# UltronAI/Depth-VO-Feat

Hardware: AMD Instinct MI355X
Metric: KITTI 256x832 stereo-seq samples/sec fwd+bwd (higher is better)
Workload: dtype f32

## Files before the change

### depth-vo-feat_amd/PoseExpNet.py

```python
from PoseExpNet_sfm import _PoseExpBase


class PoseExpNet(_PoseExpBase):

    def __init__(self, output_exp=True):
        super(PoseExpNet, self).__init__()
        self.nb_ref_imgs = 2
        self.output_exp = output_exp
        self._build(6, 6, self.nb_ref_imgs, output_exp)

    def forward(self, imgs):
        masks, pose = self._run(imgs)
        pose = pose.view(pose.size(0), 6)
        if self.training:
            return masks, pose
        return masks[0], pose
```

### depth-vo-feat_amd/PoseExpNet_sfm.py

```python
import torch
import torch.nn as nn

from dvf import lib as _L
from dvf.conv import FusedAct, FusedConv2d, FusedConvTranspose2d, SpatialMeanFn, xavier_init_

_ENC_PLANES = (16, 32, 64, 128, 256, 256, 256)
_ENC_KERNEL = (7, 5, 3, 3, 3, 3, 3)
_DEC_PLANES = (256, 128, 64, 32, 16)


class _PoseExpBase(nn.Module):

    def _build(self, in_planes, n_pose_out, nb_masks, output_exp):
        cin = in_planes
        for i, (co, k) in enumerate(zip(_ENC_PLANES, _ENC_KERNEL), start=1):
            setattr(self, f"conv{i}", nn.Sequential(FusedConv2d(cin, co, k, 2, (k - 1) // 2, _L.ACT_RELU, fuse_bwd=True), FusedAct()))
            cin = co
        self.pose_pred = FusedConv2d(_ENC_PLANES[6], n_pose_out, 1, 1, 0)
        if output_exp:
            up_in = (_ENC_PLANES[4],) + _DEC_PLANES[:-1]
            for j, lvl in enumerate(range(5, 0, -1)):
                setattr(self, f"upconv{lvl}", nn.Sequential(
                    FusedConvTranspose2d(up_in[j], _DEC_PLANES[j], 4, 2, 1, _L.ACT_RELU, fuse_bwd=True), FusedAct()))
            for lvl, ci in zip((4, 3, 2, 1), _DEC_PLANES[1:]):
                setattr(self, f"predict_mask{lvl}", FusedConv2d(ci, nb_masks, 3, 1, 1, _L.ACT_SIGMOID_AFFINE))

    def init_weights(self):
        xavier_init_(self)

    def _run(self, frames):
        outs = []
        h = frames
        for i in range(1, 8):
            h = getattr(self, f"conv{i}")[0](*h) if isinstance(h, (list, tuple)) else getattr(self, f"conv{i}")[0](h)
            outs.append(h)
        pose = SpatialMeanFn.apply(self.pose_pred(h), 0.01)
        masks = [None, None, None, None]
        if self.output_exp:
            first = frames[0] if isinstance(frames, (list, tuple)) else frames
            refs = [outs[3], outs[2], outs[1], outs[0], first]
            h = outs[4]
            ups = []
            for j, lvl in enumerate(range(5, 0, -1)):
                h = getattr(self, f"upconv{lvl}")[0](h, out_hw=(refs[j].size(2), refs[j].size(3)))
                ups.append(h)
            for lvl in (4, 3, 2, 1):
                masks[lvl - 1] = getattr(self, f"predict_mask{lvl}")(ups[5 - lvl])
        return masks, pose


class PoseExpNet(_PoseExpBase):

    def __init__(self, nb_ref_imgs=2, output_exp=True):
        super(PoseExpNet, self).__init__()
        self.nb_ref_imgs = nb_ref_imgs
        self.output_exp = output_exp
        self._build(3 * (1 + nb_ref_imgs), 6 * nb_ref_imgs, nb_ref_imgs, output_exp)

    def forward(self, target_image, ref_imgs):
        assert(len(ref_imgs) == self.nb_ref_imgs)
        frames = [target_image] + list(ref_imgs)
        if len(frames) > _L.MAX_SEGS:
            raise ValueError(f"nb_ref_imgs = {self.nb_ref_imgs}: at most {_L.MAX_SEGS - 1} reference images are supported")
        masks, pose = self._run(frames)
        pose = pose.view(pose.size(0), self.nb_ref_imgs, 6)
        if self.training:
            return masks, pose
        return masks[0], pose
```

### depth-vo-feat_amd/csrc/conv.hip

```cpp
#include "dvf_common.h"
#include "conv_op.h"
#include "conv_pipe_host.h"
#include "conv_gather.h"
#include "conv_wgrad.h"
#include "wgrad_pipe.h"

namespace {

__device__ __forceinline__ float act_grad(float g, float yv, int act, float alpha, float beta) {
    if (act == DVF_ACT_RELU) return (yv > 0.f) ? g : 0.f;
    if (act == DVF_ACT_SIGMOID_AFFINE) {
        const float sg = (yv - beta) / alpha;
        return g * alpha * sg * (1.f - sg);
    }
    return g;
}

template <bool VEC>
__global__ __launch_bounds__(256) void act_bwd_kernel(const float *__restrict__ dy, const float *__restrict__ y,
                                                      float *__restrict__ dpre, float *dbias, int C, int HW, int act,
                                                      float alpha, float beta, int chunks, float *part = nullptr, int nper = 0) {
    __shared__ float red[4];
    const int plane = blockIdx.x / chunks, chunk = blockIdx.x - plane * chunks;
    const int c = plane % C;
    const int64_t base = (int64_t)plane * HW;
    float s = 0.f;
    if (VEC) {
        typedef float f4 __attribute__((ext_vector_type(4)));
        const int HW4 = HW >> 2, per = (HW4 + chunks - 1) / chunks;
        const int beg = chunk * per, end = min(HW4, beg + per);
        const f4 *dy4 = reinterpret_cast<const f4 *>(dy + base), *y4 = reinterpret_cast<const f4 *>(y ? y + base : dy + base);
        f4 *o4 = reinterpret_cast<f4 *>(dpre ? dpre + base : nullptr);
        for (int i0 = beg + threadIdx.x; i0 < end; i0 += 1024) {
            f4 g[4], yv[4];
#pragma unroll
            for (int k = 0; k < 4; ++k) {
                const int i = i0 + 256 * k;
                if (i < end) { g[k] = dy4[i]; yv[k] = (act != DVF_ACT_NONE) ? y4[i] : g[k]; }
            }
#pragma unroll
            for (int k = 0; k < 4; ++k) {
                const int i = i0 + 256 * k;
                if (i < end) {
                    f4 r;
#pragma unroll
                    for (int e = 0; e < 4; ++e) { r[e] = act_grad(g[k][e], yv[k][e], act, alpha, beta); s += r[e]; }
                    if (dpre) o4[i] = r;
                }
            }
        }
    } else {
        const int per = (HW + chunks - 1) / chunks;
        const int beg = chunk * per, end = min(HW, beg + per);
        for (int i = beg + threadIdx.x; i < end; i += 256) {
            const float g = act_grad(dy[base + i], (act != DVF_ACT_NONE) ? y[base + i] : 0.f, act, alpha, beta);
            if (dpre) dpre[base + i] = g;
            s += g;
        }
    }
    if (dbias) {
        s = wave_sum(s);
        if ((threadIdx.x & 63) == 0) red[threadIdx.x >> 6] = s;
        __syncthreads();
        if (threadIdx.x == 0) {
            const float t = (red[0] + red[1]) + (red[2] + red[3]);
            if (part) part[(int64_t)c * nper + (plane / C) * chunks + chunk] = t;
            else atomicAdd(&dbias[c], t);
        }
    }
}

__global__ __launch_bounds__(64) void bias_finish_kernel(const float *__restrict__ part, float *dbias, int n) {
    const float *p = part + (int64_t)blockIdx.x * n;
    float s = 0.f;
    for (int i = threadIdx.x; i < n; i += 64) s += p[i];
    s = wave_sum(s);
    if (threadIdx.x == 0) dbias[blockIdx.x] += s;
}

struct TilePlan { int lsw, lsh, TGX, TGY, NT; };

TilePlan plan_tiles(int OHc, int OWc, int NT, int maxBW = 64) {
    TilePlan best{5, 0, 1, 4 * NT, NT};
    double best_cost = 1e30;
    for (int lsw = 5; lsw >= 0; --lsw) {
        const int lsh = 5 - lsw, SW = 1 << lsw, SH = 1 << lsh;
        for (int TGX = 1; TGX <= 4 * NT; TGX *= 2) {
            const int TGY = 4 * NT / TGX, BW = TGX * SW, BH = TGY * SH;
            if (BW > maxBW) continue;
            const double cov = (double)cdiv(OWc, BW) * BW * cdiv(OHc, BH) * BH;
            const double cost = cov * (1.0 + 0.02 * lsh) + 1e-3 * (BW + BH);
            if (cost < best_cost) { best_cost = cost; best = TilePlan{lsw, lsh, TGX, TGY, NT}; }
        }
    }
    return best;
}

struct GatherPlan {
    GatherArgs a;
    int MT, NT, CKH;
    size_t lds;
    dim3 grid;
    int64_t ws_floats;
    bool reduce_kpar;
};

int plan_gather(const ConvOp &op, GatherPlan &pl) {
    const ClassSpec *cls = op.cls;
    const int ncls = op.ncls, Tmax = op.Tmax, TAmax = op.TAmax, TBmax = op.TBmax, OHc = op.OHc, OWc = op.OWc;
    if (ncls < 1 || ncls > 4) return DVF_ERR_INVALID_ARG;
    GatherArgs &a = pl.a;
    a = GatherArgs{};
    for (int s = 0; s < op.nseg; ++s) a.segC[s] = op.segC[s];
    a.nseg = op.nseg; a.w_mode = op.w_mode;
    a.Mtot = op.Mtot; a.Rtot = op.Rtot; a.KK = op.KK; a.m_base = op.m_base; a.M = op.M;
    a.N = op.N; a.IH = op.IH; a.IW = op.IW; a.OH = op.OH; a.OW = op.OW;
    a.act = op.act; a.alpha = op.alpha; a.beta = op.beta;
    a.ncls = ncls; a.OS = cls[0].OS; a.IS = cls[0].IS;
    for (int i = 0, tap0 = 0; i < ncls; ++i) {
        const ClassSpec &c = cls[i];
        const int T = c.TA * c.TB;
// ... 355 lines not shown

extern "C" {

int64_t dvf_conv2d_wgrad_ws_floats(const dvf_conv_desc *d, const int *seg_channels, int nseg) {
    int rc = check_desc(d);
    if (rc) return rc;
    rc = check_segs(d, seg_channels, nseg);
    if (rc) return rc;
    int64_t need = 0;
    if (dvf_head_applicable(d, nseg)) {
        need = dvf_head_wgrad_ws_floats(d);
    } else {
        const float *const none[DVF_MAX_SEGS] = {};
        WgradPipePlan pp;
        auto plan = [&](int s, const int *qsegc, int qnseg) {
            const WgradArgs a = wgrad_args(d, none, seg_channels, s, nullptr, nullptr);
            if (plan_wgrad_pipe(a, qsegc, qnseg, true, false, pp) == DVF_OK && pp.ws_floats > need) need = pp.ws_floats;
        };
        if (!d->transposed) plan(-1, seg_channels, nseg);
        else for (int s = 0; s < nseg; ++s) plan(s, &d->C_out, 1);
    }
    const int64_t nb = dvf_act_bwd_ws_floats(d->N, d->C_out, d->H_out * d->W_out);
    return need > nb ? need : nb;
}

int dvf_conv2d_wgrad(const dvf_conv_desc *d, const float *const *in_segs, const int *seg_channels, int nseg,
                     const float *dpre, float *dw, int accumulate, float *dbias, int accumulate_dbias, float *ws,
                     int64_t ws_floats, void *stream) {
    if (!d) return DVF_ERR_INVALID_ARG;
    hipStream_t st = dvf_stream(stream);
    if (dbias && !accumulate_dbias &&
        hipMemsetAsync(dbias, 0, sizeof(float) * (size_t)(d->C_out > 0 ? d->C_out : 0), st) != hipSuccess)
        return DVF_ERR_LAUNCH;
    dvf_plan_reset();
    int rc = check_desc(d);
    if (rc) return rc;
    rc = check_segs(d, seg_channels, nseg);
    if (rc) return rc;
    if (!in_segs || !dpre || !dw) return DVF_ERR_INVALID_ARG;
    bool done = false;
    rc = wgrad_route(d, in_segs, seg_channels, nseg, dpre, dw, accumulate, dbias, &done, ws, ws_floats, st);
    if (rc || done || !dbias) return rc;
    return dvf_act_bwd(dpre, nullptr, nullptr, dbias, d->N, d->C_out, d->H_out * d->W_out, DVF_ACT_NONE, 1.f, 0.f, 1, ws, ws_floats, stream);
}

static int act_bwd_chunks(int N, int C, int HW, bool has_bias) {
    int chunks = (HW + 8191) / 8192;
    const int64_t planes = (int64_t)N * C;
    while (chunks > 1 && planes * chunks > 16384) chunks >>= 1;
    while (planes * chunks < 1024 && HW / (chunks * 2) >= 1024 && (!has_bias || (int64_t)N * chunks * 2 <= 128)) chunks *= 2;
    return chunks;
}

int64_t dvf_act_bwd_ws_floats(int N, int C, int HW) {
    if (N <= 0 || C <= 0 || HW <= 0) return DVF_ERR_INVALID_ARG;
    return (int64_t)C * N * act_bwd_chunks(N, C, HW, true);
}

int dvf_act_bwd(const float *dy, const float *y, float *dpre, float *dbias, int N, int C, int HW, int act, float alpha,
                float beta, int accumulate_dbias, float *ws, int64_t ws_floats, void *stream) {
    if (!dy || (act != DVF_ACT_NONE && !y) || N <= 0 || C <= 0 || HW <= 0) return DVF_ERR_INVALID_ARG;
    if (!dpre && !dbias) return DVF_OK;
    hipStream_t st = dvf_stream(stream);
    if (dbias && !accumulate_dbias && hipMemsetAsync(dbias, 0, sizeof(float) * C, st) != hipSuccess) return DVF_ERR_LAUNCH;
    const bool vec = (HW % 4 == 0) && ((reinterpret_cast<uintptr_t>(dy) | reinterpret_cast<uintptr_t>(y) |
                                        reinterpret_cast<uintptr_t>(dpre)) % 16 == 0);
    const int chunks = act_bwd_chunks(N, C, HW, dbias != nullptr);
    const int64_t planes = (int64_t)N * C;
    float *part = (dbias && ws && ws_floats >= dvf_act_bwd_ws_floats(N, C, HW)) ? ws : nullptr;
    if (vec) act_bwd_kernel<true><<<(unsigned)(planes * chunks), 256, 0, st>>>(dy, y, dpre, dbias, C, HW, act, alpha, beta, chunks, part, N * chunks);
    else act_bwd_kernel<false><<<(unsigned)(planes * chunks), 256, 0, st>>>(dy, y, dpre, dbias, C, HW, act, alpha, beta, chunks, part, N * chunks);
    DVF_LAUNCH_CHECK();
    if (part) {
        bias_finish_kernel<<<C, 64, 0, st>>>(part, dbias, N * chunks);
        DVF_LAUNCH_CHECK();
    }
    return DVF_OK;
}


int64_t dvf_conv2d_packed_floats(const dvf_conv_desc *d, const int *seg_channels, int nseg, int op_kind) {
    return conv_sizes(d, seg_channels, nseg, op_kind, false);
}

int64_t dvf_conv2d_ws_floats(const dvf_conv_desc *d, const int *seg_channels, int nseg, int op_kind) {
    return conv_sizes(d, seg_channels, nseg, op_kind, true);
}

int dvf_conv2d_pack(const dvf_conv_desc *d, const int *seg_channels, int nseg, int op_kind, const float *w, float *packed,
                    void *stream) {
    int rc = check_desc(d);
    if (rc) return rc;
    rc = check_segs(d, seg_channels, nseg);
    if (rc) return rc;
    if (!w || !packed) return DVF_ERR_INVALID_ARG;
    hipStream_t st = dvf_stream(stream);
    if (op_kind == 0) {
        ConvOp op;
        PipePlan pl;
        rc = make_fwd_op(d, seg_channels, nseg, op);
        if (!rc) rc = plan_pipe(op, pl);
        return rc ? rc : launch_pack(op, pl, w, packed, st);
    }
    if (op_kind != 1) return DVF_ERR_INVALID_ARG;
    return for_each_dgrad_seg(d, seg_channels, nseg, true, [&](const DgradSeg &v) -> int {
        return v.packed ? launch_pack(v.op, v.plan, w, packed + v.packed_off, st) : DVF_OK;
    });
}

int dvf_conv2d_fwd(const dvf_conv_desc *d, const float *const *in_segs, const int *seg_channels, int nseg,
                   const float *packed, const float *w, const float *bias, float *out, float *ws, int64_t ws_floats,
                   void *stream) {
    dvf_plan_reset();
    int rc = check_desc(d);
    if (rc) return rc;
    rc = check_segs(d, seg_channels, nseg);
    if (rc) return rc;
    if (!in_segs || !w || !out) return DVF_ERR_INVALID_ARG;
    for (int s = 0; s < nseg; ++s)
        if (!in_segs[s]) return DVF_ERR_INVALID_ARG;
    hipStream_t st = dvf_stream(stream);
    const ConvIO io{in_segs, bias, out, nullptr};
    ConvOp op;
// ... 91 lines not shown
```

### depth-vo-feat_amd/csrc/conv_head.hip

```cpp
#include "conv_head.h"
#include "conv_epilogue.h"

namespace {

using dvfp::apply_act;

constexpr int HT_W = 64, HT_H = 4;
constexpr int HP_W = HT_W + 2, HP_H = HT_H + 2;
constexpr int HCK = 8;
constexpr int HWK = 7;

__device__ __forceinline__ void stage_tile(float *lds, const float *__restrict__ src, int64_t plane, int nch, int H, int W,
                                           int y0, int x0) {
    for (int e = threadIdx.x; e < nch * HP_H * HP_W; e += 256) {
        const int ch = e / (HP_H * HP_W), r = e - ch * (HP_H * HP_W), py = r / HP_W, px = r - py * HP_W;
        const int y = y0 + py - 1, x = x0 + px - 1;
        lds[e] = (y >= 0 && y < H && x >= 0 && x < W) ? src[ch * plane + (int64_t)y * W + x] : 0.f;
    }
}

template <int ROWS, int MO, class WK>
__device__ __forceinline__ void taps9(const float (&v)[ROWS + 2][3], WK wk, float (&acc)[ROWS][MO]) {
#pragma unroll
    for (int m = 0; m < MO; ++m)
#pragma unroll
        for (int k = 0; k < 9; ++k) {
            const float w = wk(m, k);
#pragma unroll
            for (int r = 0; r < ROWS; ++r) acc[r][m] = fmaf(w, v[k / 3 + r][k % 3], acc[r][m]);
        }
}

constexpr int FT_H = 8;
constexpr int HEAD_MAX_SEGS = 3;
struct HeadSegs {
    const float *p[HEAD_MAX_SEGS];
    int c[HEAD_MAX_SEGS];
    int n;
};
template <int MO, int HCKT, int FTH>
__global__ __launch_bounds__(256) void head_fwd_kernel(const HeadSegs in, const float *__restrict__ w,
                                                       const float *__restrict__ bias, float *__restrict__ out, int C, int H,
                                                       int W, int tilesX, int act, float alpha, float beta, int ws_m, int ws_c,
                                                       int flip, const float *__restrict__ mask) {
    constexpr int ROWS = FTH / 4, FPH = FTH + 2, FPN = FPH * HP_W, FLD = (FPN + 255) / 256;
    extern __shared__ __attribute__((aligned(16))) float wsh[];
    float *tile = wsh + ((MO * C * 9 + 3) & ~3);
    for (int e = threadIdx.x; e < MO * C * 9; e += 256) {
        const int m = e / (C * 9), r = e - m * (C * 9), c = r / 9, k = r - c * 9;
        const float wv = w[(int64_t)m * ws_m + (int64_t)c * ws_c + (flip ? 8 - k : k)];
        if (MO == 16) wsh[(c * MO + m) * 9 + k] = wv;
        else wsh[e] = wv;
    }
    const int n = blockIdx.y, tY = blockIdx.x / tilesX, tX = blockIdx.x - tY * tilesX;
    const int y0 = tY * FTH, x0 = tX * HT_W;
    const int lx = threadIdx.x & (HT_W - 1), ly = (threadIdx.x >> 6) * ROWS;
    const int64_t plane = (int64_t)H * W;
    int soff[FLD];
#pragma unroll
    for (int i = 0; i < FLD; ++i) {
        const int e = threadIdx.x + 256 * i, py = e / HP_W, px = e - py * HP_W;
        const int y = y0 + py - 1, x = x0 + px - 1;
        soff[i] = (e < FPN && y >= 0 && y < H && x >= 0 && x < W) ? y * W + x : -1;
// ... 112 lines not shown
        }
    }
}

template <int MO>
__global__ __launch_bounds__(256) void head_dgrad_kernel(const float *__restrict__ dpre, const float *__restrict__ w,
                                                         float *__restrict__ din, int C, int H, int W, int tilesX,
                                                         const float *__restrict__ mask) {
    __shared__ float tile[MO * HP_H * HP_W];
    extern __shared__ __attribute__((aligned(16))) float wsh[];
    constexpr int WPC = (MO * 9 + 3) & ~3;
    for (int e = threadIdx.x; e < C * MO * 9; e += 256) {
        const int c = e / (MO * 9), r = e - c * (MO * 9), m = r / 9, k = r - m * 9;
        wsh[c * WPC + r] = w[((int64_t)m * C + c) * 9 + k];
    }
    const int n = blockIdx.y, tY = blockIdx.x / tilesX, tX = blockIdx.x - tY * tilesX;
    const int y0 = tY * HT_H, x0 = tX * HT_W;
    const int lx = threadIdx.x & (HT_W - 1), ly = threadIdx.x >> 6;
    const int64_t plane = (int64_t)H * W;
    stage_tile(tile, dpre + (int64_t)n * MO * plane, plane, MO, H, W, y0, x0);
    __syncthreads();
    float g[MO][9];
#pragma unroll
    for (int m = 0; m < MO; ++m)
#pragma unroll
        for (int a = 0; a < 3; ++a)
#pragma unroll
            for (int b = 0; b < 3; ++b) g[m][a * 3 + b] = tile[m * (HP_H * HP_W) + (ly + 2 - a) * HP_W + (lx + 2 - b)];
    const int y = y0 + ly, x = x0 + lx;
    if (y >= H || x >= W) return;
    const int64_t base = (int64_t)n * C * plane + (int64_t)y * W + x;
    float *dst = din + base;
    const float *mk = mask ? mask + base : nullptr;
    for (int c0 = 0; c0 < C; c0 += 4) {
        float sv[4], mv[4];
#pragma unroll
        for (int q = 0; q < 4; ++q) {
            const int c = min(c0 + q, C - 1);
            mv[q] = mk ? mk[c * plane] : 1.f;
            const float *wc = wsh + c * WPC;
            float s = 0.f;
#pragma unroll
            for (int m = 0; m < MO; ++m)
#pragma unroll
                for (int k = 0; k < 9; ++k) s = fmaf(wc[m * 9 + k], g[m][k], s);
            sv[q] = s;
        }
#pragma unroll
        for (int q = 0; q < 4; ++q)
            if (c0 + q < C) dst[(c0 + q) * plane] = (mv[q] > 0.f) ? sv[q] : 0.f;
    }
}

template <int MO>
__global__ __launch_bounds__(256) void head_wgrad_kernel(const float *__restrict__ in, const float *__restrict__ dpre,
                                                         float *dw, int N, int C, int H, int W, int tilesX, int tilesY,
                                                         float *part = nullptr) {
    __shared__ float tin[HWK * HP_H * HP_W];
    __shared__ float tdp[MO * HT_H * HT_W];
    __shared__ float red[4 * HWK * 9 * MO];
    const int c0 = blockIdx.x * HWK, nch = min(HWK, C - c0);
    const int64_t plane = (int64_t)H * W;
    const int wave = threadIdx.x >> 6, lane = threadIdx.x & 63;
    const int col_c = lane / 9, col_t = lane - col_c * 9, ta = col_t / 3, tb = col_t - ta * 3;
    const bool active = lane < nch * 9;
    float acc[MO];
#pragma unroll
    for (int m = 0; m < MO; ++m) acc[m] = 0.f;
    const int ntiles = N * tilesX * tilesY;
    for (int tile = blockIdx.y; tile < ntiles; tile += gridDim.y) {
        const int n = tile / (tilesX * tilesY), r = tile - n * (tilesX * tilesY), tY = r / tilesX, tX = r - tY * tilesX;
        const int y0 = tY * HT_H, x0 = tX * HT_W;
        __syncthreads();
        stage_tile(tin, in + ((int64_t)n * C + c0) * plane, plane, nch, H, W, y0, x0);
        for (int e = threadIdx.x; e < MO * HT_H * HT_W; e += 256) {
            const int m = e / (HT_H * HT_W), q = e - m * (HT_H * HT_W), py = q / HT_W, px = q - py * HT_W;
            const int y = y0 + py, x = x0 + px;
            tdp[e] = (y < H && x < W) ? dpre[((int64_t)n * MO + m) * plane + (int64_t)y * W + x] : 0.f;
        }
        __syncthreads();
        if (active) {
            const float *src = tin + col_c * (HP_H * HP_W) + (wave + ta) * HP_W + tb;
            const float *dp = tdp + wave * HT_W;
#pragma unroll 8
            for (int px = 0; px < HT_W; ++px) {
                const float v = src[px];
#pragma unroll
                for (int m = 0; m < MO; ++m) acc[m] = fmaf(dp[m * (HT_H * HT_W) + px], v, acc[m]);
            }
        }
    }
    if (active)
#pragma unroll
        for (int m = 0; m < MO; ++m) red[(wave * MO + m) * (HWK * 9) + lane] = acc[m];
    __syncthreads();
    if (wave == 0 && active) {
#pragma unroll
        for (int m = 0; m < MO; ++m) {
            const float s = (red[(0 * MO + m) * (HWK * 9) + lane] + red[(1 * MO + m) * (HWK * 9) + lane]) +
                            (red[(2 * MO + m) * (HWK * 9) + lane] + red[(3 * MO + m) * (HWK * 9) + lane]);
            const int64_t o = ((int64_t)m * C + c0 + col_c) * 9 + col_t;
            if (part) part[(int64_t)blockIdx.y * MO * C * 9 + o] = s;
            else atomicAdd(&dw[o], s);
        }
    }
}

__global__ __launch_bounds__(256) void head_wgrad_finish_kernel(const float *__restrict__ part, float *dw, int n, int groups) {
    const int e = blockIdx.x * 256 + threadIdx.x;
    if (e >= n) return;
    float s = 0.f;
    for (int g = 0; g < groups; ++g) s += part[(int64_t)g * n + e];
    dw[e] += s;
}


template <int CO, int K>
__global__ __launch_bounds__(256) void dconvt_s2_fwd_kernel(const float *__restrict__ in, const float *__restrict__ w,
                                                            const float *__restrict__ bias, float *__restrict__ out, int C, int H,
                                                            int W, int OH, int OW, int act, float alpha, float beta) {
    extern __shared__ __attribute__((aligned(16))) float wlds[];
    constexpr int WPC = CO * K * K;
    static_assert(WPC % 4 == 0, "weights of one input channel are read in 16-byte pieces");
    typedef float f4w __attribute__((ext_vector_type(4)));
    for (int e = threadIdx.x; e < C * WPC / 4; e += 256)
        reinterpret_cast<f4w *>(wlds)[e] = reinterpret_cast<const f4w *>(w)[e];
    __syncthreads();
    const int x = blockIdx.x * 64 + (threadIdx.x & 63), y = blockIdx.y * 4 + (threadIdx.x >> 6), n = blockIdx.z;
    const bool inside = x < W && y < H;
    const bool rok[3] = {y - 1 >= 0 && y - 1 < H, y < H, y + 1 < H}, cok[3] = {x - 1 >= 0 && x - 1 < W, x < W, x + 1 < W};
    float acc[2][2][CO];
#pragma unroll
    for (int co = 0; co < CO; ++co) {
        const float b = bias ? bias[co] : 0.f;
        acc[0][0][co] = acc[0][1][co] = acc[1][0][co] = acc[1][1][co] = b;
    }
    const int64_t plane = (int64_t)H * W;
    const float *ip = in + (int64_t)n * C * plane + (int64_t)y * W + x;
    for (int ci = 0; ci < C; ++ci) {
        float v[3][3];
#pragma unroll
        for (int r = (K == 3 ? 1 : 0); r < 3; ++r)
#pragma unroll
            for (int c = (K == 3 ? 1 : 0); c < 3; ++c) v[r][c] = (rok[r] && cok[c]) ? ip[(r - 1) * W + (c - 1)] : 0.f;
        const f4w *wc = reinterpret_cast<const f4w *>(wlds + ci * WPC);
        f4w wq[WPC / 4];
#pragma unroll
        for (int q = 0; q < WPC / 4; ++q) wq[q] = wc[q];
#pragma unroll
        for (int co = 0; co < CO; ++co) {
#pragma unroll
            for (int a = 0; a < K; ++a) {
                const int dy = (a + 1) & 1;
                const int ry = 1 + ((dy + 1 - a) >> 1);
// ... 104 lines not shown
    const int one = d->C_in;
    return dvf_head_fwd_segs(d, &in, &one, 1, w, bias, out, st);
}

bool dvf_head_wide_applicable(const dvf_conv_desc *d, int nseg) {
    return nseg >= 1 && nseg <= HEAD_MAX_SEGS && !d->transposed && d->KH == 3 && d->KW == 3 && d->stride == 1 && d->pad == 1 &&
           d->C_out == 16 && d->C_in <= 24 && d->H_out == d->H_in && d->W_out == d->W_in &&
           (int64_t)d->H_in * d->W_in >= 64 * 64 && dvf_tune("DVF_NO_HEAD") == nullptr && dvf_tune("DVF_NO_WIDE_HEAD") == nullptr;
}

int dvf_head_fwd_segs(const dvf_conv_desc *d, const float *const *in_segs, const int *seg_channels, int nseg, const float *w,
                      const float *bias, float *out, hipStream_t st) {
    HeadSegs in{};
    for (int s = 0; s < HEAD_MAX_SEGS; ++s) { in.p[s] = s < nseg ? in_segs[s] : in_segs[0]; in.c[s] = s < nseg ? seg_channels[s] : 0; }
    in.n = nseg;
    const int rc = head_fwd_launch(d->C_out, in, w, bias, out, d->C_in, d->N, d->H_in, d->W_in, d->act, d->alpha, d->beta,
                                   d->C_in * 9, 9, 0, nullptr, st);
    if (rc) return rc;
    dvf_plan_note(DVF_K_HEAD_FWD, d->C_out, nseg);
    return DVF_OK;
}

bool dvf_head_seg_dgrad_applicable(const dvf_conv_desc *d, int segc) {
    const bool narrow = segc >= 1 && segc <= 4 && d->C_out >= 4 && d->C_out * segc <= 1024;
    const bool wide = segc == 16 && d->C_out <= 24 && (int64_t)d->H_in * d->W_in >= 64 * 64 &&
                      dvf_tune("DVF_NO_WIDE_HEAD") == nullptr;
    return !d->transposed && d->KH == 3 && d->KW == 3 && d->stride == 1 && d->pad == 1 && (narrow || wide) &&
           d->H_out == d->H_in && d->W_out == d->W_in && dvf_tune("DVF_NO_HEAD") == nullptr;
}

int dvf_head_seg_dgrad(const dvf_conv_desc *d, const float *dpre, const float *w, float *din, int seg_off, int segc,
                       hipStream_t st, const float *mask) {
    const float *wseg = w + (int64_t)seg_off * 9;
    HeadSegs in{};
    for (int s = 0; s < HEAD_MAX_SEGS; ++s) { in.p[s] = dpre; in.c[s] = s == 0 ? d->C_out : 0; }
    in.n = 1;
    const int rc = head_fwd_launch(segc, in, wseg, nullptr, din, d->C_out, d->N, d->H_in, d->W_in, DVF_ACT_NONE, 1.f, 0.f, 9,
                                   d->C_in * 9, 1, mask, st);
    if (rc) return rc;
    dvf_plan_note(DVF_K_HEAD_SEG_DGRAD, segc);
    return DVF_OK;
}

int dvf_head_dgrad(const dvf_conv_desc *d, const float *dpre, const float *w, float *din, hipStream_t st, const float *mask) {
    const int tilesX = cdiv(d->W_in, HT_W), tilesY = cdiv(d->H_in, HT_H);
    const dim3 grid(tilesX * tilesY, d->N);
    HEAD_DISPATCH(d->C_out, (head_dgrad_kernel<MO><<<grid, 256, (size_t)d->C_in * ((MO * 9 + 3) & ~3) * 4, st>>>(
                                dpre, w, din, d->C_in, d->H_in, d->W_in, tilesX, mask)));
    DVF_LAUNCH_CHECK();
    dvf_plan_note(DVF_K_HEAD_DGRAD, d->C_out);
    return DVF_OK;
}

static void head_wgrad_grid(const dvf_conv_desc *d, int &tilesX, int &tilesY, int &chunks, int &groups) {
    tilesX = cdiv(d->W_in, HT_W); tilesY = cdiv(d->H_in, HT_H);
    chunks = cdiv(d->C_in, HWK);
    const int ntiles = d->N * tilesX * tilesY;
    groups = 2048 / chunks;
    if (groups < 1) groups = 1;
    if (groups > ntiles) groups = ntiles;
}

int64_t dvf_head_wgrad_ws_floats(const dvf_conv_desc *d) {
    int tilesX, tilesY, chunks, groups;
    head_wgrad_grid(d, tilesX, tilesY, chunks, groups);
    return (int64_t)groups * d->C_out * d->C_in * 9;
}

int dvf_head_wgrad(const dvf_conv_desc *d, const float *in, const float *dpre, float *dw, int accumulate, hipStream_t st,
                   float *ws, int64_t ws_floats) {
    if (!accumulate && hipMemsetAsync(dw, 0, sizeof(float) * (size_t)d->C_out * d->C_in * 9, st) != hipSuccess)
        return DVF_ERR_LAUNCH;
    int tilesX, tilesY, chunks, groups;
    head_wgrad_grid(d, tilesX, tilesY, chunks, groups);
    const dim3 grid(chunks, groups);
    float *part = (ws && ws_floats >= dvf_head_wgrad_ws_floats(d)) ? ws : nullptr;
    HEAD_DISPATCH(d->C_out, (head_wgrad_kernel<MO><<<grid, 256, 0, st>>>(in, dpre, dw, d->N, d->C_in, d->H_in, d->W_in, tilesX,
                                                                        tilesY, part)));
    DVF_LAUNCH_CHECK();
    if (part) {
        const int n = d->C_out * d->C_in * 9;
        head_wgrad_finish_kernel<<<(n + 255) / 256, 256, 0, st>>>(part, dw, n, groups);
        DVF_LAUNCH_CHECK();
    }
    dvf_plan_note(DVF_K_HEAD_WGRAD, d->C_out, part ? 1 : 0);
    return DVF_OK;
}
```

### depth-vo-feat_amd/dvf/steps.py

```python

import torch

import loss_functions as LF
import loss_functions_sfm as LS
from dvf import lib as L
from dvf.conv import reciprocal


POSE_STREAM = True


def _side_by_side(aux_fn, main_fn):
    if L.SERIALIZE or not POSE_STREAM:
        m_out = main_fn()
        return aux_fn(), m_out
    cur = torch.cuda.current_stream()
    aux = L.aux_stream(cur.device)
    aux.wait_stream(cur)
    m_out = main_fn()
    with torch.cuda.stream(aux):
        a_out = aux_fn()
    cur.wait_stream(aux)

    def _mark(t):
        if torch.is_tensor(t):
            t.record_stream(cur)
        elif isinstance(t, (list, tuple)):
            for x in t:
                _mark(x)
    _mark(a_out)
    return a_out, m_out


def _identity_share(counts, n_views):
    return counts[n_views:2 * n_views].sum() / counts.sum()


def unsupervise_losses(depth_net, pose_net, batch, feat_extractor=None, img_scale=0.004, smooth_weight=10.0,
                       feat_weight=0.1, depth_eps=1e-4, ssim_weight=0.0, ssim_c1=1e-4, ssim_c2=9e-4, min_reprojection=False,
                       auto_mask=False, normalized_smoothness=False):
    counts = []
    R2, R1, L2 = batch["img_R2"], batch["img_R1"], batch["img_L2"]
    (_, T_2to1), disps = _side_by_side(lambda: pose_net((R2, R1)), lambda: depth_net(R2))
    inv_depth = disps[0]
    depth = reciprocal(inv_depth, depth_eps).squeeze(1)
    img_loss = LF.photometric_reconstruction_loss(R2, R1, L2, depth, T_2to1, batch["T_R2L"], batch["K"], batch["Kinv"],
                                                  img_scale=img_scale,
                                                  ssim_weight=ssim_weight, ssim_c1=ssim_c1, ssim_c2=ssim_c2,
                                                  min_reprojection=min_reprojection, auto_mask=auto_mask,
                                                  selection_counts=counts)
    if normalized_smoothness:
        smooth = LF.normalized_smooth_loss(inv_depth, R2, img_scale=img_scale)
    else:
        smooth = LF.smooth_loss(depth.unsqueeze(1))
    terms = {"img": img_loss.detach(), "smooth": smooth.detach()}
    if auto_mask:
        terms["automask"] = _identity_share(counts[0], 2)
    loss = img_loss + smooth_weight * smooth
    if feat_extractor is not None:
        b = R2.size(0)
        feat = feat_extractor(torch.cat((L2, R2, R1), dim=0))
        f_L2, f_R2, f_R1 = feat[:b], feat[b:2 * b], feat[2 * b:]
        feat_loss = LF.photometric_reconstruction_loss(f_R2, f_R1, f_L2, depth, T_2to1, batch["T_R2L"], batch["K"],
                                                       batch["Kinv"])
        loss = img_loss + feat_weight * feat_loss + smooth_weight * smooth
        terms["feat"] = feat_loss.detach()
    terms["total"] = loss.detach()
    return loss, terms


def depth_only_losses(depth_net, batch, img_scale=0.004, smooth_weight=10.0, depth_eps=1e-4):
    R2, L2 = batch["img_R2"], batch["img_L2"]
    depth = reciprocal(depth_net(R2)[0], depth_eps)
    from dvf.ops import PhotoLossFn
    photo = PhotoLossFn.apply(R2, depth.squeeze(1), batch["T_R2L"].unsqueeze(0).contiguous(), batch["K"], batch["Kinv"], None,
                              (0, float(img_scale)), L2)
    smooth = LF.smooth_loss(depth)
    loss = photo + smooth_weight * smooth
    return loss, {"img": photo.detach(), "smooth": smooth.detach(), "total": loss.detach()}


def train_sfm_losses(disp_net, pose_exp_net, batch, w1=1.0, w2=0.0, w3=0.1, smooth_factor=2.0,
                     rotation_mode="euler", padding_mode="zeros", feat_extractor=None, feat_weight=0.1,
                     ssim_weight=0.0, ssim_c1=1e-4, ssim_c2=9e-4, min_reprojection=False, auto_mask=False,
                     full_res_multiscale=False, normalized_smoothness=False):
    if min_reprojection and w2 > 0:
        raise ValueError("min_reprojection leaves the explainability mask out of the photometric term: w2 must be 0")
    tgt = batch["img_R2"]
    refs = [batch["img_R1"], batch["img_L2"]] + list(batch.get("extra_refs", []))[: pose_exp_net.nb_ref_imgs - 2]
    (masks, pose), disparities = _side_by_side(lambda: pose_exp_net(tgt, refs), lambda: disp_net(tgt))
    depth = [reciprocal(d, 0.0) for d in disparities]
    counts = []
    photo_depth, photo_masks = depth, masks
    if full_res_multiscale:
        hw = tgt.shape[2:]
        photo_depth = LS.full_resolution(disparities, hw, recip_eps=0.0)
        if not min_reprojection:
            photo_masks = LS.full_resolution(masks, hw)
    l1 = LS.photometric_reconstruction_loss(tgt, refs, batch["K"], batch["Kinv"], photo_depth,
                                            [None] * len(depth) if min_reprojection else photo_masks, pose,
                                            rotation_mode, padding_mode, ssim_weight=ssim_weight, ssim_c1=ssim_c1,
                                            ssim_c2=ssim_c2, min_reprojection=min_reprojection, auto_mask=auto_mask,
                                            selection_counts=counts)
    if normalized_smoothness:
        l3 = LS.normalized_smooth_loss(disparities, tgt, smooth_factor)
    else:
        l3 = LS.smooth_loss(depth, smooth_factor)
    l4 = torch.nn.functional.mse_loss(pose[:, 1], batch["T_R2L"])
    loss = w1 * l1 + w3 * l3 + l4
    terms = {"photo": l1.detach(), "smooth": l3.detach(), "lr": l4.detach()}
    if auto_mask:
        terms["automask"] = _identity_share(counts[0], len(refs))
    if w2 > 0:
        l2 = LS.explainability_loss(masks)
        loss = loss + w2 * l2
        terms["exp"] = l2.detach()
    if feat_extractor is not None:
        b = tgt.size(0)
        feat = feat_extractor(torch.cat((refs[1], tgt, refs[0]), dim=0))
        f_L2, f_R2, f_R1 = feat[:b], feat[b:2 * b], feat[2 * b:]
        lf = LF.photometric_reconstruction_loss(f_R2, f_R1, f_L2, depth[0].squeeze(1), pose[:, 0], pose[:, 1], batch["K"],
                                                batch["Kinv"], rotation_mode, padding_mode)
        loss = loss + feat_weight * lf
        terms["feat"] = lf.detach()
    terms["total"] = loss.detach()
    return loss, terms


def unsupervise_dvo_losses(depth_net, pose_net, batch, img_scale=0.004, smooth_weight=10.0, depth_eps=1e-4,
                           normalized_smoothness=False):
    from dvf.ops import PhotoLossFn
    R2, R1, L2 = batch["img_R2"], batch["img_R1"], batch["img_L2"]
    (_, T_2to1), disps = _side_by_side(lambda: pose_net((R2, R1)), lambda: depth_net(R2))
    inv_depth = disps[0]
    depth = reciprocal(inv_depth, depth_eps)
    pose = torch.stack((batch["T_R2L"], T_2to1), dim=0)
    photo = PhotoLossFn.apply(R2, depth.squeeze(1), pose, batch["K"], batch["Kinv"], None,
                              (L.POSE_SE3 | L.PIXEL_COORDS, float(img_scale)), L2, R1)
    smooth = LF.normalized_smooth_loss(inv_depth, R2, img_scale=img_scale) if normalized_smoothness else LF.smooth_loss(depth)
    loss = photo + smooth_weight * smooth
    return loss, {"photo": photo.detach(), "smooth": smooth.detach(), "total": loss.detach()}


def paper_losses(depth_net, pose_net, batch, feat_extractor=None, img_scale=0.004, smooth_weight=10.0, feat_weight=0.1,
                 depth_eps=1e-4):
    import loss_functions_caffe as LC
    R2, R1, L2 = batch["img_R2"], batch["img_R1"], batch["img_L2"]
    (_, T_2to1), disps = _side_by_side(lambda: pose_net((R2, R1)), lambda: depth_net(R2))
    inv_depth = disps[0]
    depth = reciprocal(inv_depth, depth_eps)
    poses = (batch["T_R2L_se3"], T_2to1)
    photo = LC.abs_warp_loss(R2, (L2, R1), depth, poses, batch["K"], batch["Kinv"], img_scale=img_scale)
    smooth = LC.edge_aware_smooth_loss(inv_depth, R2, img_scale=img_scale)
    loss = photo + smooth_weight * smooth
    terms = {"photo": photo.detach(), "smooth": smooth.detach()}
    if feat_extractor is not None:
        b = R2.size(0)
        with torch.no_grad():
            feat = feat_extractor(torch.cat((L2, R2, R1), dim=0))
        f_L2, f_R2, f_R1 = feat[:b], feat[b:2 * b], feat[2 * b:]
        lf = LC.abs_warp_loss(f_R2, (f_L2, f_R1), depth, poses, batch["K"], batch["Kinv"])
        loss = loss + feat_weight * lf
        terms["feat"] = lf.detach()
    terms["total"] = loss.detach()
    return loss, terms
```

Before: 615.9.

## Skip unused mask decoder, add bias-sum kernel, rewrite head wgrad as register sliding window

The stereo-sequence loss paths now call the pose net with need_masks=False, so the upconv/mask decoder is not run when its masks are discarded. A dedicated wide bias-sum reduction kernel handles the bias-only backward case (no activation, no dpre) with its own chunking. The 3x3 head weight-gradient kernel is rewritten from LDS tiles into a per-thread register sliding window over row segments with vectorized loads and tunable channel and row grouping. Together these remove wasted forward/backward work and cut reduction overhead, at the cost of more registers and new tuning heuristics.

```diff
diff --git a/depth-vo-feat_amd/PoseExpNet.py b/depth-vo-feat_amd/PoseExpNet.py
--- a/depth-vo-feat_amd/PoseExpNet.py
+++ b/depth-vo-feat_amd/PoseExpNet.py
@@ -9,8 +9,8 @@
         self.output_exp = output_exp
         self._build(6, 6, self.nb_ref_imgs, output_exp)
 
-    def forward(self, imgs):
-        masks, pose = self._run(imgs)
+    def forward(self, imgs, need_masks=True):
+        masks, pose = self._run(imgs, need_masks)
         pose = pose.view(pose.size(0), 6)
         if self.training:
             return masks, pose
diff --git a/depth-vo-feat_amd/PoseExpNet_sfm.py b/depth-vo-feat_amd/PoseExpNet_sfm.py
--- a/depth-vo-feat_amd/PoseExpNet_sfm.py
+++ b/depth-vo-feat_amd/PoseExpNet_sfm.py
@@ -28,7 +28,7 @@
     def init_weights(self):
         xavier_init_(self)
 
-    def _run(self, frames):
+    def _run(self, frames, need_masks=True):
         outs = []
         h = frames
         for i in range(1, 8):
@@ -36,7 +36,7 @@
             outs.append(h)
         pose = SpatialMeanFn.apply(self.pose_pred(h), 0.01)
         masks = [None, None, None, None]
-        if self.output_exp:
+        if self.output_exp and need_masks:
             first = frames[0] if isinstance(frames, (list, tuple)) else frames
             refs = [outs[3], outs[2], outs[1], outs[0], first]
             h = outs[4]
@@ -57,12 +57,12 @@
         self.output_exp = output_exp
         self._build(3 * (1 + nb_ref_imgs), 6 * nb_ref_imgs, nb_ref_imgs, output_exp)
 
-    def forward(self, target_image, ref_imgs):
+    def forward(self, target_image, ref_imgs, need_masks=True):
         assert(len(ref_imgs) == self.nb_ref_imgs)
         frames = [target_image] + list(ref_imgs)
         if len(frames) > _L.MAX_SEGS:
             raise ValueError(f"nb_ref_imgs = {self.nb_ref_imgs}: at most {_L.MAX_SEGS - 1} reference images are supported")
-        masks, pose = self._run(frames)
+        masks, pose = self._run(frames, need_masks)
         pose = pose.view(pose.size(0), self.nb_ref_imgs, 6)
         if self.training:
             return masks, pose
diff --git a/depth-vo-feat_amd/csrc/conv.hip b/depth-vo-feat_amd/csrc/conv.hip
--- a/depth-vo-feat_amd/csrc/conv.hip
+++ b/depth-vo-feat_amd/csrc/conv.hip
@@ -67,6 +67,54 @@
             if (part) part[(int64_t)c * nper + (plane / C) * chunks + chunk] = t;
             else atomicAdd(&dbias[c], t);
         }
+    }
+}
+
+template <bool VEC>
+__global__ __launch_bounds__(1024) void bias_sum_kernel(const float *__restrict__ dy, float *dbias, int C, int HW, int chunks,
+                                                        float *part, int nper) {
+    __shared__ float red[16];
+    constexpr int U = 8, UT = 4;
+    typedef typename std::conditional<VEC, float __attribute__((ext_vector_type(4))), float>::type V;
+    const int T = blockDim.x;
+    const int plane = blockIdx.x / chunks, chunk = blockIdx.x - plane * chunks;
+    const int c = plane % C;
+    const int E = VEC ? HW >> 2 : HW, per = (E + chunks - 1) / chunks;
+    const int beg = chunk * per, n = min(E, beg + per) - beg;
+    const V *p = reinterpret_cast<const V *>(dy + (int64_t)plane * HW) + beg;
+    const V zero = {};
+    V a0 = zero, a1 = zero;
+    int i = threadIdx.x;
+    for (; i + T * (U - 1) < n; i += T * U) {
+        V g[U];
+#pragma unroll
+        for (int k = 0; k < U; ++k) g[k] = p[i + T * k];
+#pragma unroll
+        for (int k = 0; k < U; k += 2) { a0 += g[k]; a1 += g[k + 1]; }
+    }
+    for (; i < n; i += T * UT) {
+        V g[UT];
+#pragma unroll
+        for (int k = 0; k < UT; ++k) g[k] = p[min(i + T * k, n - 1)];
+#pragma unroll
+        for (int k = 0; k < UT; ++k) a0 += (i + T * k < n) ? g[k] : zero;
+    }
+    a0 += a1;
+    float s;
+    if constexpr (VEC) s = (a0[0] + a0[1]) + (a0[2] + a0[3]);
+    else s = a0;
+    s = wave_sum(s);
+    if (T > 64) {
+        if ((threadIdx.x & 63) == 0) red[threadIdx.x >> 6] = s;
+        __syncthreads();
+        if (threadIdx.x == 0) {
+            s = red[0];
+            for (int w = 1; w < (T >> 6); ++w) s += red[w];
+        }
+    }
+    if (threadIdx.x == 0) {
+        if (part) part[(int64_t)c * nper + (plane / C) * chunks + chunk] = s;
+        else atomicAdd(&dbias[c], s);
     }
 }
 
@@ -528,9 +576,18 @@
     return chunks;
 }
 
+static int bias_sum_chunks(int N, int C, int HW) {
+    int target = 256;
+    if (const char *t = dvf_tune("DVF_BIAS_BLOCKS")) target = atoi(t);
+    int chunks = 1;
+    while ((int64_t)N * C * chunks * 2 <= target && HW / (chunks * 2) >= 8192) chunks *= 2;
+    return chunks;
+}
+
 int64_t dvf_act_bwd_ws_floats(int N, int C, int HW) {
     if (N <= 0 || C <= 0 || HW <= 0) return DVF_ERR_INVALID_ARG;
-    return (int64_t)C * N * act_bwd_chunks(N, C, HW, true);
+    const int a = act_bwd_chunks(N, C, HW, true), b = bias_sum_chunks(N, C, HW);
+    return (int64_t)C * N * (a > b ? a : b);
 }
 
 int dvf_act_bwd(const float *dy, const float *y, float *dpre, float *dbias, int N, int C, int HW, int act, float alpha,
@@ -541,10 +598,16 @@
     if (dbias && !accumulate_dbias && hipMemsetAsync(dbias, 0, sizeof(float) * C, st) != hipSuccess) return DVF_ERR_LAUNCH;
     const bool vec = (HW % 4 == 0) && ((reinterpret_cast<uintptr_t>(dy) | reinterpret_cast<uintptr_t>(y) |
                                         reinterpret_cast<uintptr_t>(dpre)) % 16 == 0);
-    const int chunks = act_bwd_chunks(N, C, HW, dbias != nullptr);
+    const bool sums_only = !dpre && act == DVF_ACT_NONE;
+    const int chunks = sums_only ? bias_sum_chunks(N, C, HW) : act_bwd_chunks(N, C, HW, dbias != nullptr);
     const int64_t planes = (int64_t)N * C;
     float *part = (dbias && ws && ws_floats >= dvf_act_bwd_ws_floats(N, C, HW)) ? ws : nullptr;
-    if (vec) act_bwd_kernel<true><<<(unsigned)(planes * chunks), 256, 0, st>>>(dy, y, dpre, dbias, C, HW, act, alpha, beta, chunks, part, N * chunks);
+    if (sums_only) {
+        const int per = ((vec ? HW >> 2 : HW) + chunks - 1) / chunks;
+        const int threads = per <= 256 ? 64 : per <= 8192 ? 256 : 1024;
+        if (vec) bias_sum_kernel<true><<<(unsigned)(planes * chunks), threads, 0, st>>>(dy, dbias, C, HW, chunks, part, N * chunks);
+        else bias_sum_kernel<false><<<(unsigned)(planes * chunks), threads, 0, st>>>(dy, dbias, C, HW, chunks, part, N * chunks);
+    } else if (vec) act_bwd_kernel<true><<<(unsigned)(planes * chunks), 256, 0, st>>>(dy, y, dpre, dbias, C, HW, act, alpha, beta, chunks, part, N * chunks);
     else act_bwd_kernel<false><<<(unsigned)(planes * chunks), 256, 0, st>>>(dy, y, dpre, dbias, C, HW, act, alpha, beta, chunks, part, N * chunks);
     DVF_LAUNCH_CHECK();
     if (part) {
diff --git a/depth-vo-feat_amd/csrc/conv_head.hip b/depth-vo-feat_amd/csrc/conv_head.hip
--- a/depth-vo-feat_amd/csrc/conv_head.hip
+++ b/depth-vo-feat_amd/csrc/conv_head.hip
@@ -8,7 +8,6 @@
 constexpr int HT_W = 64, HT_H = 4;
 constexpr int HP_W = HT_W + 2, HP_H = HT_H + 2;
 constexpr int HCK = 8;
-constexpr int HWK = 7;
 
 __device__ __forceinline__ void stage_tile(float *lds, const float *__restrict__ src, int64_t plane, int nch, int H, int W,
                                            int y0, int x0) {
@@ -227,54 +226,114 @@
     }
 }
 
-template <int MO>
+template <bool VEC>
+__device__ __forceinline__ void hw_load4(const float *__restrict__ p, int x0, int W, bool ok, float (&v)[4]) {
+    if (VEC) {
+        typedef float f4 __attribute__((ext_vector_type(4)));
+        f4 t = {0.f, 0.f, 0.f, 0.f};
+        if (ok) t = *reinterpret_cast<const f4 *>(p);
+#pragma unroll
+        for (int j = 0; j < 4; ++j) v[j] = t[j];
+    } else {
+#pragma unroll
+        for (int j = 0; j < 4; ++j) v[j] = (ok && x0 + j < W) ? p[j] : 0.f;
+    }
+}
+
+template <int MO, int CCH, bool VEC>
 __global__ __launch_bounds__(256) void head_wgrad_kernel(const float *__restrict__ in, const float *__restrict__ dpre,
-                                                         float *dw, int N, int C, int H, int W, int tilesX, int tilesY,
-                                                         float *part = nullptr) {
-    __shared__ float tin[HWK * HP_H * HP_W];
-    __shared__ float tdp[MO * HT_H * HT_W];
-    __shared__ float red[4 * HWK * 9 * MO];
-    const int c0 = blockIdx.x * HWK, nch = min(HWK, C - c0);
+                                                         float *dw, int C, int H, int W, int RS, int xgroups, int segs,
+                                                         int64_t units, float *part = nullptr) {
+    constexpr int A = CCH * 9 * MO;
+    __shared__ float red[4 * A];
+    const int c0 = blockIdx.x * CCH;
     const int64_t plane = (int64_t)H * W;
+    const int upi = segs * xgroups;
+    float acc[CCH][9][MO];
+#pragma unroll
+    for (int c = 0; c < CCH; ++c)
+#pragma unroll
+        for (int t = 0; t < 9; ++t)
+#pragma unroll
+            for (int m = 0; m < MO; ++m) acc[c][t][m] = 0.f;
+    for (int64_t ub = blockIdx.y; ub * 256 < units; ub += gridDim.y) {
+        const int64_t u = ub * 256 + threadIdx.x;
+        const bool live = u < units;
+        const int n = live ? (int)(u / upi) : 0, q = live ? (int)(u - (int64_t)n * upi) : 0;
+        const int seg = q / xgroups, xg = q - seg * xgroups;
+        const int y0 = seg * RS, y1 = min(H, y0 + RS), x0 = xg * 4;
+        const float *ip = in + ((int64_t)n * C + c0) * plane + x0;
+        const float *dp = dpre + (int64_t)n * MO * plane + x0;
+        const bool lok = x0 > 0, rok = x0 + 4 < W;
+        auto load_in = [&](int r, float (&x)[CCH][6]) __attribute__((always_inline)) {
+            const bool ok = live && r >= 0 && r < H;
+            const int64_t ro = (int64_t)r * W;
+#pragma unroll
+            for (int c = 0; c < CCH; ++c) {
+                const bool okc = ok && c0 + c < C;
+                const float *p = ip + c * plane + ro;
+                float v[4];
+                hw_load4<VEC>(p, x0, W, okc, v);
+                x[c][0] = (okc && lok) ? p[-1] : 0.f;
+#pragma unroll
+                for (int j = 0; j < 4; ++j) x[c][1 + j] = v[j];
+                x[c][5] = (okc && rok) ? p[4] : 0.f;
+            }
+        };
+        auto load_dp = [&](int y, float (&g)[MO][4]) __attribute__((always_inline)) {
+            const bool ok = live && y >= y0 && y < y1;
+#pragma unroll
+            for (int m = 0; m < MO; ++m) hw_load4<VEC>(dp + m * plane + (int64_t)y * W, x0, W, ok, g[m]);
+        };
+        float d[3][MO][4], dn[MO][4], xc[CCH][6], xn[CCH][6];
+#pragma unroll
+        for (int m = 0; m < MO; ++m)
+#pragma unroll
+            for (int j = 0; j < 4; ++j) d[0][m][j] = d[1][m][j] = 0.f;
+        load_dp(y0, d[2]);
+        load_in(y0 - 1, xc);
+        for (int i = 0; i < RS + 2; ++i) {
+            const int r = y0 - 1 + i;
+            load_in(i + 1 < RS + 2 ? r + 1 : H, xn);
+            load_dp(r + 2, dn);
+#pragma unroll
+            for (int c = 0; c < CCH; ++c)
+#pragma unroll
+                for (int ta = 0; ta < 3; ++ta)
+#pragma unroll
+                    for (int tb = 0; tb < 3; ++tb)
+#pragma unroll
+                        for (int m = 0; m < MO; ++m)
+#pragma unroll
+                            for (int j = 0; j < 4; ++j)
+                                acc[c][ta * 3 + tb][m] = fmaf(d[2 - ta][m][j], xc[c][j + tb], acc[c][ta * 3 + tb][m]);
+#pragma unroll
+            for (int m = 0; m < MO; ++m)
+#pragma unroll
+                for (int j = 0; j < 4; ++j) { d[0][m][j] = d[1][m][j]; d[1][m][j] = d[2][m][j]; d[2][m][j] = dn[m][j]; }
+#pragma unroll
+            for (int c = 0; c < CCH; ++c)
+#pragma unroll
+                for (int j = 0; j < 6; ++j) xc[c][j] = xn[c][j];
+        }
+    }
     const int wave = threadIdx.x >> 6, lane = threadIdx.x & 63;
-    const int col_c = lane / 9, col_t = lane - col_c * 9, ta = col_t / 3, tb = col_t - ta * 3;
-    const bool active = lane < nch * 9;
-    float acc[MO];
-#pragma unroll
-    for (int m = 0; m < MO; ++m) acc[m] = 0.f;
-    const int ntiles = N * tilesX * tilesY;
-    for (int tile = blockIdx.y; tile < ntiles; tile += gridDim.y) {
-        const int n = tile / (tilesX * tilesY), r = tile - n * (tilesX * tilesY), tY = r / tilesX, tX = r - tY * tilesX;
-        const int y0 = tY * HT_H, x0 = tX * HT_W;
-        __syncthreads();
-        stage_tile(tin, in + ((int64_t)n * C + c0) * plane, plane, nch, H, W, y0, x0);
-        for (int e = threadIdx.x; e < MO * HT_H * HT_W; e += 256) {
-            const int m = e / (HT_H * HT_W), q = e - m * (HT_H * HT_W), py = q / HT_W, px = q - py * HT_W;
-            const int y = y0 + py, x = x0 + px;
-            tdp[e] = (y < H && x < W) ? dpre[((int64_t)n * MO + m) * plane + (int64_t)y * W + x] : 0.f;
-        }
-        __syncthreads();
-        if (active) {
-            const float *src = tin + col_c * (HP_H * HP_W) + (wave + ta) * HP_W + tb;
-            const float *dp = tdp + wave * HT_W;
-#pragma unroll 8
-            for (int px = 0; px < HT_W; ++px) {
-                const float v = src[px];
-#pragma unroll
-                for (int m = 0; m < MO; ++m) acc[m] = fmaf(dp[m * (HT_H * HT_W) + px], v, acc[m]);
-            }
-        }
-    }
-    if (active)
-#pragma unroll
-        for (int m = 0; m < MO; ++m) red[(wave * MO + m) * (HWK * 9) + lane] = acc[m];
+#pragma unroll
+    for (int c = 0; c < CCH; ++c)
+#pragma unroll
+        for (int t = 0; t < 9; ++t)
+#pragma unroll
+            for (int m = 0; m < MO; ++m) {
+                const float s = wave_sum(acc[c][t][m]);
+                if (lane == 0) red[wave * A + (c * 9 + t) * MO + m] = s;
+            }
     __syncthreads();
-    if (wave == 0 && active) {
-#pragma unroll
-        for (int m = 0; m < MO; ++m) {
-            const float s = (red[(0 * MO + m) * (HWK * 9) + lane] + red[(1 * MO + m) * (HWK * 9) + lane]) +
-                            (red[(2 * MO + m) * (HWK * 9) + lane] + red[(3 * MO + m) * (HWK * 9) + lane]);
-            const int64_t o = ((int64_t)m * C + c0 + col_c) * 9 + col_t;
+    const int a = threadIdx.x;
+    if (a < A) {
+        const int c = a / (9 * MO), q = a - c * (9 * MO), t = q / MO, m = q - t * MO;
+        if (c0 + c < C) {
+            const float s = (red[a] + red[A + a]) + (red[2 * A + a] + red[3 * A + a]);
+            const int64_t o = ((int64_t)m * C + c0 + c) * 9 + t;
             if (part) part[(int64_t)blockIdx.y * MO * C * 9 + o] = s;
             else atomicAdd(&dw[o], s);
         }
@@ -485,35 +544,51 @@
     return DVF_OK;
 }
 
-static void head_wgrad_grid(const dvf_conv_desc *d, int &tilesX, int &tilesY, int &chunks, int &groups) {
-    tilesX = cdiv(d->W_in, HT_W); tilesY = cdiv(d->H_in, HT_H);
-    chunks = cdiv(d->C_in, HWK);
-    const int ntiles = d->N * tilesX * tilesY;
-    groups = 2048 / chunks;
+struct HeadWgradGrid { int cch, RS, xgroups, segs, chunks, groups; int64_t units; };
+static HeadWgradGrid head_wgrad_grid(const dvf_conv_desc *d) {
+    HeadWgradGrid g;
+    g.xgroups = cdiv(d->W_in, 4);
+    auto blocks = [&](int cch, int rs) {
+        return (int64_t)cdiv(d->C_in, cch) * (((int64_t)d->N * cdiv(d->H_in, rs) * g.xgroups + 255) / 256);
+    };
+    const int min_blocks = 400, max_blocks = 1024;
+    g.cch = (d->C_out <= 2 && blocks(4, 8) >= 512) ? 4 : 2;
+    g.RS = 8;
+    if (const char *t = dvf_tune("DVF_HEAD_WG_CCH")) g.cch = (atoi(t) == 4 && d->C_out <= 2) ? 4 : 2;
+    while (g.RS > 2 && blocks(g.cch, g.RS) < min_blocks) g.RS >>= 1;
+    if (const char *t = dvf_tune("DVF_HEAD_WG_RS")) g.RS = atoi(t) > 0 ? atoi(t) : g.RS;
+    g.segs = cdiv(d->H_in, g.RS);
+    g.units = (int64_t)d->N * g.segs * g.xgroups;
+    g.chunks = cdiv(d->C_in, g.cch);
+    const int64_t nub = (g.units + 255) / 256;
+    int64_t groups = max_blocks / g.chunks;
     if (groups < 1) groups = 1;
-    if (groups > ntiles) groups = ntiles;
+    if (groups > nub) groups = nub;
+    g.groups = (int)groups;
+    return g;
 }
 
 int64_t dvf_head_wgrad_ws_floats(const dvf_conv_desc *d) {
-    int tilesX, tilesY, chunks, groups;
-    head_wgrad_grid(d, tilesX, tilesY, chunks, groups);
-    return (int64_t)groups * d->C_out * d->C_in * 9;
+    return (int64_t)head_wgrad_grid(d).groups * d->C_out * d->C_in * 9;
 }
 
 int dvf_head_wgrad(const dvf_conv_desc *d, const float *in, const float *dpre, float *dw, int accumulate, hipStream_t st,
                    float *ws, int64_t ws_floats) {
     if (!accumulate && hipMemsetAsync(dw, 0, sizeof(float) * (size_t)d->C_out * d->C_in * 9, st) != hipSuccess)
         return DVF_ERR_LAUNCH;
-    int tilesX, tilesY, chunks, groups;
-    head_wgrad_grid(d, tilesX, tilesY, chunks, groups);
-    const dim3 grid(chunks, groups);
+    const HeadWgradGrid g = head_wgrad_grid(d);
+    const dim3 grid(g.chunks, g.groups);
     float *part = (ws && ws_floats >= dvf_head_wgrad_ws_floats(d)) ? ws : nullptr;
-    HEAD_DISPATCH(d->C_out, (head_wgrad_kernel<MO><<<grid, 256, 0, st>>>(in, dpre, dw, d->N, d->C_in, d->H_in, d->W_in, tilesX,
-                                                                        tilesY, part)));
+    const bool vec = d->W_in % 4 == 0 && ((reinterpret_cast<uintptr_t>(in) | reinterpret_cast<uintptr_t>(dpre)) & 15) == 0;
+#define HEAD_WGRAD_GO(CCH, VEC) head_wgrad_kernel<MO, CCH, VEC><<<grid, 256, 0, st>>>(in, dpre, dw, d->C_in, d->H_in, d->W_in, g.RS, g.xgroups, g.segs, g.units, part)
+    HEAD_DISPATCH(d->C_out, {
+        if (MO <= 2 && g.cch == 4) { if (vec) HEAD_WGRAD_GO((MO <= 2 ? 4 : 2), true); else HEAD_WGRAD_GO((MO <= 2 ? 4 : 2), false); }
+        else { if (vec) HEAD_WGRAD_GO(2, true); else HEAD_WGRAD_GO(2, false); } });
+#undef HEAD_WGRAD_GO
     DVF_LAUNCH_CHECK();
     if (part) {
         const int n = d->C_out * d->C_in * 9;
-        head_wgrad_finish_kernel<<<(n + 255) / 256, 256, 0, st>>>(part, dw, n, groups);
+        head_wgrad_finish_kernel<<<(n + 255) / 256, 256, 0, st>>>(part, dw, n, g.groups);
         DVF_LAUNCH_CHECK();
     }
     dvf_plan_note(DVF_K_HEAD_WGRAD, d->C_out, part ? 1 : 0);
diff --git a/depth-vo-feat_amd/dvf/steps.py b/depth-vo-feat_amd/dvf/steps.py
--- a/depth-vo-feat_amd/dvf/steps.py
+++ b/depth-vo-feat_amd/dvf/steps.py
@@ -32,6 +32,13 @@
     return a_out, m_out
 
 
+def _pose_only(pose_net, frames):
+    from PoseExpNet_sfm import _PoseExpBase
+    if isinstance(getattr(pose_net, "module", pose_net), _PoseExpBase):
+        return pose_net(frames, need_masks=False)
+    return pose_net(frames)
+
+
 def _identity_share(counts, n_views):
     return counts[n_views:2 * n_views].sum() / counts.sum()
 
@@ -41,7 +48,7 @@
                        auto_mask=False, normalized_smoothness=False):
     counts = []
     R2, R1, L2 = batch["img_R2"], batch["img_R1"], batch["img_L2"]
-    (_, T_2to1), disps = _side_by_side(lambda: pose_net((R2, R1)), lambda: depth_net(R2))
+    (_, T_2to1), disps = _side_by_side(lambda: _pose_only(pose_net, (R2, R1)), lambda: depth_net(R2))
     inv_depth = disps[0]
     depth = reciprocal(inv_depth, depth_eps).squeeze(1)
     img_loss = LF.photometric_reconstruction_loss(R2, R1, L2, depth, T_2to1, batch["T_R2L"], batch["K"], batch["Kinv"],
@@ -131,7 +138,7 @@
                            normalized_smoothness=False):
     from dvf.ops import PhotoLossFn
     R2, R1, L2 = batch["img_R2"], batch["img_R1"], batch["img_L2"]
-    (_, T_2to1), disps = _side_by_side(lambda: pose_net((R2, R1)), lambda: depth_net(R2))
+    (_, T_2to1), disps = _side_by_side(lambda: _pose_only(pose_net, (R2, R1)), lambda: depth_net(R2))
     inv_depth = disps[0]
     depth = reciprocal(inv_depth, depth_eps)
     pose = torch.stack((batch["T_R2L"], T_2to1), dim=0)
@@ -146,7 +153,7 @@
                  depth_eps=1e-4):
     import loss_functions_caffe as LC
     R2, R1, L2 = batch["img_R2"], batch["img_R1"], batch["img_L2"]
-    (_, T_2to1), disps = _side_by_side(lambda: pose_net((R2, R1)), lambda: depth_net(R2))
+    (_, T_2to1), disps = _side_by_side(lambda: _pose_only(pose_net, (R2, R1)), lambda: depth_net(R2))
     inv_depth = disps[0]
     depth = reciprocal(inv_depth, depth_eps)
     poses = (batch["T_R2L_se3"], T_2to1)
```

Result: faster. 647.8, median of 6 (+5.2%).
